# segasai/rvspecfit

Hardware: AMD Instinct MI355X
Metric: spectra/sec (CCF+chi2 grid) DESI 3-arm (higher is better)
Workload: dtype f64

## Files before the change

rvspecfit_amd/csrc/ccf_fft.hip:

```cpp
#include "common.h"

#define XC_NT 512
#define XC_NTW(n2) ((n2) >> 3)

__device__ __forceinline__ double2 cmul(double2 a, double2 b) {
  return make_double2(a.x * b.x - a.y * b.y, a.x * b.y + a.y * b.x);
}
__device__ __forceinline__ double2 cadd(double2 a, double2 b) {
  return make_double2(a.x + b.x, a.y + b.y);
}
__device__ __forceinline__ double2 csub(double2 a, double2 b) {
  return make_double2(a.x - b.x, a.y - b.y);
}
template <int SIGN>
__device__ __forceinline__ double2 cmuli(double2 a) {
  return (SIGN > 0) ? make_double2(-a.y, a.x) : make_double2(a.y, -a.x);
}

__host__ __device__ inline int xc_plan(int log2n, int *rad) {
  int n = 0, l = log2n;
  while (l >= 3) {
    rad[n++] = 8;
    l -= 3;
  }
// ... 44 lines not shown
  a[4] = csub(e0, o0);
  a[1] = cadd(e1, w1o);
  a[5] = csub(e1, w1o);
  a[2] = cadd(e2, w2o);
  a[6] = csub(e2, w2o);
  a[3] = cadd(e3, w3o);
  a[7] = csub(e3, w3o);
}

template <int SIGN>
__device__ __forceinline__ double2 twid(const double2 *__restrict__ tw, int e,
                                        int nfft) {
  const int half = nfft >> 1;
  double2 w = (e < half) ? tw[e] : tw[e - half];
  if (e >= half) {
    w.x = -w.x;
    w.y = -w.y;
  }
  if (SIGN < 0) w.y = -w.y;
  return w;
}

#ifdef RVS_XC_TIMING
__device__ unsigned long long xc_dbg[16];
#define XC_T(i)                                        \
  do {                                                 \
    __syncthreads();                                   \
    if (threadIdx.x == 0) {                            \
      const unsigned long long t_ = wall_clock64();    \
      atomicAdd(&xc_dbg[i], t_ - t_prev);              \
      t_prev = t_;                                     \
    }                                                  \
  } while (0)
extern "C" int rvs_dbg_read_xc(unsigned long long *out) {
  return hipMemcpyFromSymbol(out, HIP_SYMBOL(xc_dbg), sizeof(xc_dbg)) ==
                 hipSuccess
             ? 0
             : -1;
}
#else
#define XC_T(i)
#endif

template <int NT>
__device__ __forceinline__ void xc_fill_twiddles(double2 *a, int n2,
                                                 const double2 *__restrict__ tw) {
  const int ntw = XC_NTW(n2);
  if ((ntw & 63) == 0) {
    const int lane = threadIdx.x & 63;
    for (int i0 = (threadIdx.x >> 6) * 64; i0 < ntw; i0 += NT) {
      __builtin_amdgcn_global_load_lds(
          (const __attribute__((address_space(1))) void *)(tw + 2 * (i0 + lane)),
          (__attribute__((address_space(3))) void *)(a + n2 + i0), 16, 0, 0);
    }
    return;
  }
  for (int i = threadIdx.x; i < ntw; i += NT) a[n2 + i] = tw[2 * i];
}

struct XcMasks {
  unsigned g, b0, b7;
};
template <int NT>
__device__ __forceinline__ XcMasks xc_load_masks(const uint8_t *__restrict__ prune,
                                                 int n2) {
  XcMasks m = {0u, 0u, 0u};
  if (prune && (n2 >> 3) <= NT) {
    const int t = threadIdx.x, B = t >> 3;
    if (t < (n2 >> 3)) m.g = prune[(n2 >> 6) + t];
    if (B < (n2 >> 6)) {
      m.b0 = prune[(n2 >> 6) + 8 * B];
      m.b7 = prune[(n2 >> 6) + 8 * B + 7];
    }
  }
// ... 128 lines not shown
          const double2 w2 = cmul(w1, w1), w3 = cmul(w2, w1);
          v1 = cmul(v1, w1);
          v2 = cmul(v2, w2);
          v3 = cmul(v3, w3);
        }
        a[base] = v0;
        a[base + Mp] = v1;
        a[base + 2 * Mp] = v2;
        a[base + 3 * Mp] = v3;
      } else {
        const double2 v0 = a[base], v1 = a[base + Mp];
        double2 d = csub(v0, v1);
        if (Mp > 1) d = cmul(d, twid<SIGN>(tw, r << tws, nfft));
        a[base] = cadd(v0, v1);
        a[base + Mp] = d;
      }
    }
    lgM = lgMp;
  }
  __syncthreads();
}

__device__ __forceinline__ int fft_pos(int f, int log2n) {
  int pos = 0, lgm = log2n;
  while (lgm > 0) {
    const int lgr = lgm >= 3 ? 3 : lgm;
    lgm -= lgr;
    pos += (f & ((1 << lgr) - 1)) << lgm;
    f >>= lgr;
  }
  return pos;
}

__global__ void __launch_bounds__(XC_NT)
    ccf_rfft_kernel(const double *__restrict__ proc_spec,
                    const double *__restrict__ proc_ivar, int nfft, int log2n,
                    const double2 *__restrict__ tw, double2 *__restrict__ work) {
  extern __shared__ double2 fa[];
  const int b = blockIdx.x, which = blockIdx.y, tid = threadIdx.x;
  const int n2 = nfft >> 1;
  const double *ps = proc_spec + (int64_t)b * nfft;
  const double *pi = proc_ivar + (int64_t)b * nfft;
  xc_fill_twiddles<XC_NT>(fa, n2, tw);
  for (int n = tid; n < n2; n += XC_NT) {
    double x0, x1;
    if (which == 0) {
      x0 = ps[2 * n] * pi[2 * n];
      x1 = ps[2 * n + 1] * pi[2 * n + 1];
    } else {
      x0 = pi[2 * n];
      x1 = pi[2 * n + 1];
    }
    fa[n] = make_double2(x0, x1);
  }
  fft_lds<-1, XC_NT>(fa, log2n, tw);
  double2 *out = work + ((int64_t)b * 2 + which) * (n2 + 1);
  for (int k = tid; k <= n2; k += XC_NT) {
    double2 X;
    if (k == 0 || k == n2) {
      const double2 z0 = fa[0];
      X = make_double2(k == 0 ? z0.x + z0.y : z0.x - z0.y, 0.0);
    } else {
      const double2 zk = fa[fft_pos(k, log2n)];
      const double2 zm = fa[fft_pos(n2 - k, log2n)];
      const double2 e = make_double2(zk.x + zm.x, zk.y - zm.y);
      const double2 d = make_double2(zk.x - zm.x, zk.y + zm.y);
      const double2 q = cmul(twid<-1>(tw, k, nfft), d);
      X = make_double2(0.5 * (e.x + q.y), 0.5 * (e.y - q.x));
    }
    out[k] = make_double2(X.x, -X.y);
  }
}

#define XB_NT 512

__device__ __forceinline__ bool xc_job(unsigned bid, int T, int B, int G, int &b,
                                       int &t) {
  const int xcd = bid & 7;
  const int slot = bid >> 3;
  const int tt = slot % G;
  const int q = slot / G;
  b = q % B;
  const int g = q / B;
  t = xcd + 8 * (g * G + tt);
  return t < T;
}
__host__ inline int64_t xc_nblocks(int T, int B, int G) {
  const int ntx = (T + 7) >> 3;
  const int ngrp = (ntx + G - 1) / G;
  return 8ll * ngrp * G * B;
}
__host__ inline int xc_group(int T, int nfft) {
  const int64_t per_t = 2ll * ((nfft >> 1) + 1) * 16;
  if (per_t * T <= (16ll << 20)) return 0;
#ifndef XC_GROUP_BYTES
#define XC_GROUP_BYTES (2ll << 20)
#endif
  int G = (int)(XC_GROUP_BYTES / per_t);
  const int ntx = (T + 7) >> 3;
  if (G < 1) G = 1;
  if (G > ntx) G = ntx;
// ... 169 lines not shown
#define XW_NT 1024
#define XW_HALF 512

template <int SIGN, int LOG2N>
__device__ __forceinline__ void xw_pass(double2 *a, const double2 *T1, int p, int t,
                                        const double2 *Tc = nullptr) {
  const int lgM = LOG2N - 3 * p, lgMp = lgM - 3, Mp = 1 << lgMp;
  const int tws = LOG2N + 1 - lgM;
  const int blk = t >> lgMp, r = t & (Mp - 1);
  const int base = (blk << lgM) + r;
  double2 v[8];
#pragma unroll
  for (int j = 0; j < 8; j++) v[j] = a[base + Mp * j];
  dft8<SIGN>(v);
  if (Mp > 1) {
    double2 w1 = Tc ? Tc[r] : T1[r << (tws - 1)];
    if (SIGN < 0) w1.y = -w1.y;
    v[1] = cmul(v[1], w1);
    const double2 w2 = cmul(w1, w1);
    v[2] = cmul(v[2], w2);
    double2 wc = cmul(w2, w1);
    v[3] = cmul(v[3], wc);
    const double2 w4 = cmul(w2, w2);
    v[4] = cmul(v[4], w4);
    v[7] = cmul(v[7], cmul(w4, wc));
    wc = cmul(w4, w1);
    v[5] = cmul(v[5], wc);
    v[6] = cmul(v[6], cmul(w4, w2));
  }
#pragma unroll
  for (int q = 0; q < 8; q++) a[base + Mp * q] = v[q];
}

template <int LOG2N, bool RATIO>
__global__ void __launch_bounds__(XW_NT)
    ccf_xcorr_ws_kernel(const double2 *__restrict__ work,
                        const double2 *__restrict__ tfft,
                        const double2 *__restrict__ tfft2, int T,
                        const double2 *__restrict__ tw,
                        const int32_t *__restrict__ lag_pos,
                        const double *__restrict__ lag_vel, int nlag,
                        const int32_t *__restrict__ ilo,
                        const double *__restrict__ vgrid, int nvel, double beta,
                        const uint8_t *__restrict__ prune,
                        double *__restrict__ chisq) {
  extern __shared__ double2 fa[];
  constexpr int log2n = LOG2N, n2 = 1 << LOG2N, nfft = 2 * n2, npair = n2 / 2;
  constexpr int NPP = npair / XW_HALF;
  constexpr bool P12 = (LOG2N == 12);
  static_assert(LOG2N == 12 || LOG2N == 11, "plans 8,8,8,8 and 8,8,8,4 only");
  auto img = [&](int i) -> double2 * { return fa + (i & 1) * n2; };
  const double2 *T1 = fa + 2 * n2;
  double *c0 = reinterpret_cast<double *>(fa + 2 * n2 + XC_NTW(n2));
  double2 *T1c = fa + 2 * n2 + XC_NTW(n2) + ((nlag + 1) >> 1);
  double *cA = reinterpret_cast<double *>(T1c + 73);
  const int TI = RATIO ? 2 * T : T;
  const int b = blockIdx.x, tid = threadIdx.x;
  const bool producer = tid >= XW_HALF;
  const int pt = tid & (XW_HALF - 1);
  const double inv_n = 1.0 / nfft;
  if (P12 && tid < 72)
    T1c[tid] = tid < 64 ? tw[2 * (tid << 3)] : tw[2 * ((tid - 64) << (log2n - 6))];
  xc_fill_twiddles<XW_NT>(fa + n2, n2, tw);
  XcMasks pmask = {0u, 0u, 0u};
  bool bad = !P12;
  if (P12 && !producer) {
    pmask = xc_load_masks<XW_HALF>(prune, n2);
    const int pos8 = pt & 7;
    const unsigned m = pmask.g;
    bad = m != 0 && !((pos8 == 0 && m == 0x01u) || (pos8 == 7 && m == 0x80u));
  }
  const bool fold = !__syncthreads_or(bad);
  const double2 *Sc = work + ((int64_t)b * 2) * (n2 + 1);
  const double2 *Vc = Sc + (n2 + 1);
  typedef int v4i_t __attribute__((ext_vector_type(4)));
  auto ld = [](const __amdgpu_buffer_rsrc_t &r, int off) {
    const v4i_t v = __builtin_amdgcn_raw_buffer_load_b128(r, off, 0, 0);
    return make_double2(__hiloint2double(v.y, v.x), __hiloint2double(v.w, v.z));
  };
  const int nbytes = (n2 + 1) * 16;
  if (producer) {
    double2 Sk[NPP], Vk[NPP], Sm[NPP], Vm[NPP];
#pragma unroll
    for (int u = 0; u < NPP; u++) {
      const int k = 1 + pt + u * XW_HALF, m = n2 - k;
      Sk[u] = Sc[k], Vk[u] = Vc[k], Sm[u] = Sc[m], Vm[u] = Vc[m];
    }
    const __amdgpu_buffer_rsrc_t rT = __builtin_amdgcn_make_buffer_rsrc(
        (void *)tw, 0, (npair + 1) * 16, 0x00020000);
    double2 op[2][5];
    auto issue = [&](int t, int u, double2 *o) {
      const int tt = RATIO ? (t >> 1) : t;
      const __amdgpu_buffer_rsrc_t rF = __builtin_amdgcn_make_buffer_rsrc(
          (void *)(((RATIO && (t & 1)) ? tfft2 : tfft) + (int64_t)tt * (n2 + 1)), 0,
          nbytes, 0x00020000);
      const __amdgpu_buffer_rsrc_t rF2 = __builtin_amdgcn_make_buffer_rsrc(
          (void *)(tfft2 + (int64_t)tt * (n2 + 1)), 0, nbytes, 0x00020000);
      int ptv = pt;
      asm volatile("" : "+v"(ptv));
      const int k = 1 + ptv + u * XW_HALF;
      const int ok = k * 16, om = (n2 - k) * 16;
      if (RATIO) {
        o[0] = ld(rF, ok);
        o[2] = ld(rF, om);
      } else {
        o[0] = ld(rF, ok), o[1] = ld(rF2, ok);
        o[2] = ld(rF, om), o[3] = ld(rF2, om);
      }
      o[4] = ld(rT, ok);
    };
    double2 dc[4];
    auto form = [&](double2 *dst, int u, const double2 *o, int tcur) {
      int ptv = pt;
      asm volatile("" : "+v"(ptv));
      const int k = 1 + ptv + u * XW_HALF, m = n2 - k;
      double2 Xk, Xm;
      if (RATIO) {
        const bool second = (tcur & 1) != 0;
        Xk = cmul(o[0], second ? Vk[u] : Sk[u]);
        Xm = cmul(o[2], second ? Vm[u] : Sm[u]);
      } else {
        const double2 p1 = cmul(o[0], Sk[u]), p2 = cmul(o[1], Vk[u]);
        Xk = make_double2(p2.x - 2 * p1.x, p2.y - 2 * p1.y);
        const double2 q1 = cmul(o[2], Sm[u]), q2 = cmul(o[3], Vm[u]);
        Xm = make_double2(q2.x - 2 * q1.x, q2.y - 2 * q1.y);
      }
      const double2 e = make_double2(Xk.x + Xm.x, Xk.y - Xm.y);
      const double2 d = make_double2(Xk.x - Xm.x, Xk.y + Xm.y);
      const double2 q = cmul(o[4], d);
      dst[k] = make_double2(e.x - q.y, e.y + q.x);
      if (m != k) dst[m] = make_double2(e.x + q.y, -e.y + q.x);
      if (u == NPP - 1 && ptv == 0) {
        double xk, xm;
        if (RATIO) {
          const bool second = (tcur & 1) != 0;
          xk = cmul(second ? dc[1] : dc[0], second ? Vc[0] : Sc[0]).x;
          xm = cmul(second ? dc[3] : dc[2], second ? Vc[n2] : Sc[n2]).x;
        } else {
          const double2 a1 = cmul(dc[0], Sc[0]), a2 = cmul(dc[1], Vc[0]);
          const double2 b1 = cmul(dc[2], Sc[n2]), b2 = cmul(dc[3], Vc[n2]);
          xk = a2.x - 2 * a1.x, xm = b2.x - 2 * b1.x;
        }
        dst[0] = make_double2(xk + xm, xk - xm);
      }
    };
    const int nbar = (P12 && fold) ? 4 : 5;
    issue(0, 0, op[0]);
    if (NPP == 2) issue(0, 1, op[1]);
    for (int it = -1; it < TI; it++) {
      const int tn = it + 1;
      if (tn < TI) {
        double2 *dst = img(tn);
        {
          const int tt = RATIO ? (tn >> 1) : tn;
          const double2 *Fp = tfft + (int64_t)tt * (n2 + 1);
          const double2 *F2p = tfft2 + (int64_t)tt * (n2 + 1);
          dc[0] = Fp[0], dc[1] = F2p[0], dc[2] = Fp[n2], dc[3] = F2p[n2];
        }
        if (NPP == 2) {
#pragma unroll
          for (int u = 0; u < 2; u++) {
            form(dst, u, op[u], tn);
            if (tn + 1 < TI) issue(tn + 1, u, op[u]);
            __syncthreads();
          }
        } else {
#pragma unroll
          for (int u = 0; u < NPP; u++) {
            if (u + 1 < NPP)
              issue(tn, u + 1, op[(u + 1) & 1]);
            else if (tn + 1 < TI)
              issue(tn + 1, 0, op[(u + 1) & 1]);
            form(dst, u, op[u & 1], tn);
            __syncthreads();
          }
        }
        for (int q = NPP; q < nbar; q++) __syncthreads();
      } else {
        for (int q = 0; q < nbar; q++) __syncthreads();
      }
    }
    return;
  }
  const int tvx = min(pt, nvel - 1);
  const int pre_pos = lag_pos[min(pt, nlag - 1)];
  const int pre_lo = ilo[tvx];
  const double pre_xg = vgrid[tvx];
  const double pre_x0 = lag_vel[pre_lo], pre_x1 = lag_vel[pre_lo + 1];
  for (int it = -1; it < TI; it++) {
    if (it < 0) {
      const int nbar = (P12 && fold) ? 4 : 5;
      for (int q = 0; q < nbar; q++) __syncthreads();
      continue;
    }
    double2 *a = img(it);
    double *out = chisq + ((int64_t)b * T + (RATIO ? (it >> 1) : it)) * nvel;
    double pre_old = 0;
    if (beta != 0.0) pre_old = out[tvx];
    if (pt < (n2 >> 3)) xw_pass<1, LOG2N>(a, T1, 0, pt);
    __syncthreads();
    if (pt < (n2 >> 3)) xw_pass<1, LOG2N>(a, T1, 1, pt, P12 ? T1c : nullptr);
    __syncthreads();
    if (!P12) {
      if (pt < (n2 >> 3)) xw_pass<1, LOG2N>(a, T1, 2, pt);
      __syncthreads();
      {
        const int base = pt << 2;
        double2 v0 = a[base], v1 = a[base + 1], v2 = a[base + 2], v3 = a[base + 3];
        dft4<1>(v0, v1, v2, v3);
        a[base] = v0, a[base + 1] = v1, a[base + 2] = v2, a[base + 3] = v3;
      }
      __syncthreads();
    } else if (fold) {
      const int s = pt & 7;
      const int B = pt >> 3;
      const unsigned m0 = pmask.b0 & 1u, m63 = pmask.b7 >> 7;
      if (m0 | m63) {
        double2 v[8];
#pragma unroll
        for (int j = 0; j < 8; j++) v[j] = a[B * 64 + s + 8 * j];
        dft8<1>(v);
        double2 w = T1c[64 + s];
        w.y = -w.y;
        double2 x63 = cmul(v[7], w), x0 = v[0];
        auto sum8 = [](double x) {
          x += dpp_get<0xb1, 0xf, 0xf>(x);
          x += dpp_get<0x4e, 0xf, 0xf>(x);
          x += dpp_get<0x141, 0xf, 0xf>(x);
          return x;
        };
        if (m0) {
          x0.x = sum8(x0.x);
          x0.y = sum8(x0.y);
          if (s == 0) a[B * 64] = x0;
        }
        if (m63) {
          x63.x = sum8(x63.x);
          x63.y = sum8(x63.y);
          if (s == 0) a[B * 64 + 63] = x63;
        }
      }
      __syncthreads();
    } else {
      {
        const int blk = pt >> 3, r = pt & 7, base = (blk << 6) + r;
        const unsigned mask = prune[blk];
        if (mask != 0) {
          double2 v[8];
#pragma unroll
          for (int j = 0; j < 8; j++) v[j] = a[base + 8 * j];
          dft8<1>(v);
          double2 wp[8];
          wp[0] = make_double2(1.0, 0.0);
          wp[1] = T1[r << (log2n + 1 - 6 - 1)];
          wp[2] = cmul(wp[1], wp[1]);
          wp[3] = cmul(wp[2], wp[1]);
          wp[4] = cmul(wp[2], wp[2]);
          wp[7] = cmul(wp[4], wp[3]);
          wp[5] = cmul(wp[4], wp[1]);
          wp[6] = cmul(wp[4], wp[2]);
#pragma unroll
          for (int q = 0; q < 8; q++)
            if (mask & (1u << q))
              a[base + 8 * q] = (q == 0) ? v[0] : cmul(v[q], wp[q]);
        }
      }
      __syncthreads();
      {
        const unsigned mask = pmask.g;
        if (mask != 0) {
          const int base = pt << 3;
          double2 v[8];
#pragma unroll
          for (int j = 0; j < 8; j++) v[j] = a[base + j];
          dft8<1>(v);
#pragma unroll
          for (int q = 0; q < 8; q++)
            if (mask & (1u << q)) a[base + q] = v[q];
        }
      }
      __syncthreads();
    }
    if (RATIO) {
      if (pt < nlag) {
        const double c = reinterpret_cast<const double *>(a)[pre_pos] * inv_n;
        if (it & 1)
          c0[pt] = -cA[pt] * cA[pt] / c;
        else
          cA[pt] = c;
      }
    } else if (pt < nlag) {
      c0[pt] = reinterpret_cast<const double *>(a)[pre_pos] * inv_n;
    }
    __syncthreads();
    if ((!RATIO || (it & 1)) && pt < nvel) {
      const double sl = (c0[pre_lo + 1] - c0[pre_lo]) / (pre_x1 - pre_x0);
      const double val = sl * (pre_xg - pre_x0) + c0[pre_lo];
      out[pt] = (beta != 0.0) ? beta * pre_old + val : val;
    }
  }
}

__global__ void __launch_bounds__(XW_NT)
    ccf_xcorr_ws2_kernel(const double2 *__restrict__ work,
                         const double2 *__restrict__ tfft,
                         const double2 *__restrict__ tfft2, int T,
                         const double2 *__restrict__ tw,
                         const int32_t *__restrict__ lag_pos,
                         const double *__restrict__ lag_vel, int nlag,
                         const int32_t *__restrict__ ilo,
                         const double *__restrict__ vgrid, int nvel, double beta,
                         double *__restrict__ chisq) {
  extern __shared__ double2 fa[];
  constexpr int LOG2N = 11, n2 = 1 << LOG2N, nfft = 2 * n2, npair = n2 / 2;
  constexpr int NBAR = 5;
  auto img = [&](int i, int j) -> double2 * { return fa + (((i & 1) << 1) + j) * n2; };
  const double2 *T1 = fa + 4 * n2;
  double *c0 = reinterpret_cast<double *>(fa + 4 * n2 + XC_NTW(n2));
  const int b = blockIdx.x, tid = threadIdx.x;
  const bool producer = tid >= XW_HALF;
  const int pt = tid & (XW_HALF - 1);
  const double inv_n = 1.0 / nfft;
  xc_fill_twiddles<XW_NT>(fa + 3 * n2, n2, tw);
  const double2 *Sc = work + ((int64_t)b * 2) * (n2 + 1);
  const double2 *Vc = Sc + (n2 + 1);
  typedef int v4i_t __attribute__((ext_vector_type(4)));
  auto ld = [](const __amdgpu_buffer_rsrc_t &r, int off) {
    const v4i_t v = __builtin_amdgcn_raw_buffer_load_b128(r, off, 0, 0);
    return make_double2(__hiloint2double(v.y, v.x), __hiloint2double(v.w, v.z));
  };
  const int nbytes = (n2 + 1) * 16;
  const int NIT = (T + 1) >> 1;
  __syncthreads();
  if (producer) {
    double2 Sk[2], Vk[2], Sm[2], Vm[2];
#pragma unroll
    for (int u = 0; u < 2; u++) {
      const int k = 1 + pt + u * XW_HALF, m = n2 - k;
      Sk[u] = Sc[k], Vk[u] = Vc[k], Sm[u] = Sc[m], Vm[u] = Vc[m];
    }
    const __amdgpu_buffer_rsrc_t rT = __builtin_amdgcn_make_buffer_rsrc(
        (void *)tw, 0, (npair + 1) * 16, 0x00020000);
    double2 op[2][5];
    auto issue = [&](int t, int u, double2 *o) {
      const __amdgpu_buffer_rsrc_t rF = __builtin_amdgcn_make_buffer_rsrc(
          (void *)(tfft + (int64_t)t * (n2 + 1)), 0, nbytes, 0x00020000);
      const __amdgpu_buffer_rsrc_t rF2 = __builtin_amdgcn_make_buffer_rsrc(
          (void *)(tfft2 + (int64_t)t * (n2 + 1)), 0, nbytes, 0x00020000);
      const int k = 1 + pt + u * XW_HALF;
      const int ok = k * 16, om = (n2 - k) * 16;
      o[0] = ld(rF, ok), o[1] = ld(rF2, ok);
      o[2] = ld(rF, om), o[3] = ld(rF2, om);
      o[4] = ld(rT, ok);
    };
    auto form = [&](double2 *dst, int t, int u, const double2 *o) {
      const int k = 1 + pt + u * XW_HALF, m = n2 - k;
      const double2 p1 = cmul(o[0], Sk[u]), p2 = cmul(o[1], Vk[u]);
      const double2 Xk = make_double2(p2.x - 2 * p1.x, p2.y - 2 * p1.y);
      const double2 q1 = cmul(o[2], Sm[u]), q2 = cmul(o[3], Vm[u]);
      const double2 Xm = make_double2(q2.x - 2 * q1.x, q2.y - 2 * q1.y);
      const double2 e = make_double2(Xk.x + Xm.x, Xk.y - Xm.y);
      const double2 d = make_double2(Xk.x - Xm.x, Xk.y + Xm.y);
      const double2 q = cmul(o[4], d);
      dst[k] = make_double2(e.x - q.y, e.y + q.x);
      if (m != k) dst[m] = make_double2(e.x + q.y, -e.y + q.x);
      if (u == 1 && pt == 0) {
        const double2 *Fp = tfft + (int64_t)t * (n2 + 1);
        const double2 *F2p = tfft2 + (int64_t)t * (n2 + 1);
        const double2 a1 = cmul(Fp[0], Sc[0]), a2 = cmul(F2p[0], Vc[0]);
        const double2 b1 = cmul(Fp[n2], Sc[n2]), b2 = cmul(F2p[n2], Vc[n2]);
        const double xk = a2.x - 2 * a1.x, xm = b2.x - 2 * b1.x;
        dst[0] = make_double2(xk + xm, xk - xm);
      }
    };
    auto tq = [&](int i, int q) { return min(2 * i + (q >> 1), T - 1); };
    issue(tq(0, 0), 0, op[0]);
    for (int it = -1; it < NIT; it++) {
      const int in = it + 1;
      if (in < NIT) {
#pragma unroll
        for (int q = 0; q < 4; q++) {
          if (q + 1 < 4)
            issue(tq(in, q + 1), (q + 1) & 1, op[(q + 1) & 1]);
          else if (in + 1 < NIT)
            issue(tq(in + 1, 0), 0, op[(q + 1) & 1]);
          form(img(in, q >> 1), tq(in, q), q & 1, op[q & 1]);
          __syncthreads();
        }
        __syncthreads();
      } else {
        for (int q = 0; q < NBAR; q++) __syncthreads();
      }
    }
    return;
  }
  const int j = pt >> 8, bt = pt & 255;
  int pre_pos[1], dummy = 0;
  (void)dummy;
  pre_pos[0] = lag_pos[min(pt, nlag - 1)];
  const int tvx = min(pt, nvel - 1);
  const int pre_lo = ilo[tvx];
  const double pre_xg = vgrid[tvx];
  const double pre_x0 = lag_vel[pre_lo], pre_x1 = lag_vel[pre_lo + 1];
  for (int it = -1; it < NIT; it++) {
    if (it < 0) {
      for (int q = 0; q < NBAR; q++) __syncthreads();
      continue;
    }
    double2 *a = img(it, j);
    const int t0 = 2 * it, t1 = min(2 * it + 1, T - 1);
    const bool two = (2 * it + 1 < T);
    double *out0 = chisq + ((int64_t)b * T + t0) * nvel;
    double *out1 = chisq + ((int64_t)b * T + t1) * nvel;
    double old0 = 0, old1 = 0;
    if (beta != 0.0) {
      old0 = out0[tvx];
      old1 = out1[tvx];
    }
    xw_pass<1, LOG2N>(a, T1, 0, bt);
    __syncthreads();
    xw_pass<1, LOG2N>(a, T1, 1, bt);
    __syncthreads();
    xw_pass<1, LOG2N>(a, T1, 2, bt);
    __syncthreads();
#pragma unroll
    for (int h = 0; h < 2; h++) {
      const int base = (bt + 256 * h) << 2;
      double2 v0 = a[base], v1 = a[base + 1], v2 = a[base + 2], v3 = a[base + 3];
// ... 19 lines not shown
    }
  }
}

extern "C" int rvs_ccf_xcorr(const double *proc_spec, const double *proc_ivar,
                             int nfft, int B, const double *tfft,
                             const double *tfft2, int T, const double *twid_,
                             int continuum, const int32_t *lag_pos,
                             const double *lag_vel, int nlag, const int32_t *ilo,
                             const double *vgrid, int nvel, double beta,
                             const uint8_t *prune, double *chisq, double *work,
                             void *stream) {
  int log2n = 0;
  while ((2 << log2n) < nfft) log2n++;
  if ((2 << log2n) != nfft || nfft < 64 || nfft > 16384) return RVS_E_ARG;
  if (B < 1 || T < 1 || T > 65535 || nlag < 2 || nvel < 1) return RVS_E_ARG;
  const int n2 = nfft >> 1;
  const size_t shm1 = sizeof(double2) * (size_t)(n2 + XC_NTW(n2));
  const size_t shm2 = shm1 + sizeof(double) * 2 * (size_t)nlag;
  if (shm2 > 159 * 1024) return RVS_E_ARG;
  hipStream_t st = rvs_stream(stream);
  const double2 *tw = reinterpret_cast<const double2 *>(twid_);
  static bool attr_set = false;
  if (!attr_set) {
    (void)hipFuncSetAttribute((const void *)ccf_rfft_kernel,
                              hipFuncAttributeMaxDynamicSharedMemorySize,
                              159 * 1024);
    (void)hipFuncSetAttribute((const void *)ccf_xcorr_kernel,
                              hipFuncAttributeMaxDynamicSharedMemorySize,
                              159 * 1024);
    (void)hipGetLastError();
    attr_set = true;
  }
  hipLaunchKernelGGL(ccf_rfft_kernel, dim3(B, 2), dim3(XC_NT), shm1, st,
                     proc_spec, proc_ivar, nfft, log2n, tw,
                     reinterpret_cast<double2 *>(work));
  RVS_LAUNCH_CHECK();
  const int G = xc_group(T, nfft);
  {
    const bool ws_on = rvs_opt(RVS_OPT_XC_WS) != 0;
    const bool p12 = (nfft == 8192 && prune), p11 = (nfft == 4096);
    if (ws_on && (p12 || p11) && nlag <= XW_HALF && nvel <= XW_HALF && T >= 2) {
      static bool ws_attr = false;
      if (!ws_attr) {
        (void)hipFuncSetAttribute((const void *)ccf_xcorr_ws_kernel<12, false>,
                                  hipFuncAttributeMaxDynamicSharedMemorySize,
                                  159 * 1024);
        (void)hipFuncSetAttribute((const void *)ccf_xcorr_ws_kernel<12, true>,
                                  hipFuncAttributeMaxDynamicSharedMemorySize,
                                  159 * 1024);
        (void)hipFuncSetAttribute((const void *)ccf_xcorr_ws_kernel<11, true>,
                                  hipFuncAttributeMaxDynamicSharedMemorySize,
                                  159 * 1024);
        (void)hipFuncSetAttribute((const void *)ccf_xcorr_ws2_kernel,
                                  hipFuncAttributeMaxDynamicSharedMemorySize,
                                  159 * 1024);
        (void)hipGetLastError();
        ws_attr = true;
      }
      const size_t shmw = sizeof(double2) * (size_t)(2 * n2 + XC_NTW(n2)) +
                          sizeof(double) * (size_t)nlag +
                          sizeof(double2) * (72 + 1) +
                          (continuum ? 0 : sizeof(double) * (size_t)nlag);
#define RVS_XW_ARGS                                                                 \
  reinterpret_cast<const double2 *>(work), reinterpret_cast<const double2 *>(tfft),  \
      reinterpret_cast<const double2 *>(tfft2), T, tw, lag_pos, lag_vel, nlag, ilo,  \
      vgrid, nvel, beta, prune, chisq
      if (!continuum) {
        if (p12)
          hipLaunchKernelGGL((ccf_xcorr_ws_kernel<12, true>), dim3(B), dim3(XW_NT), shmw,
                             st, RVS_XW_ARGS);
        else
          hipLaunchKernelGGL((ccf_xcorr_ws_kernel<11, true>), dim3(B), dim3(XW_NT), shmw,
                             st, RVS_XW_ARGS);
        RVS_LAUNCH_CHECK();
        return 0;
      }
      if (p12)
        hipLaunchKernelGGL((ccf_xcorr_ws_kernel<12, false>), dim3(B), dim3(XW_NT), shmw, st,
                           reinterpret_cast<const double2 *>(work),
                           reinterpret_cast<const double2 *>(tfft),
                           reinterpret_cast<const double2 *>(tfft2), T, tw, lag_pos,
                           lag_vel, nlag, ilo, vgrid, nvel, beta, prune, chisq);
      else
        hipLaunchKernelGGL(ccf_xcorr_ws2_kernel, dim3(B), dim3(XW_NT),
                           sizeof(double2) * (size_t)(4 * n2 + XC_NTW(n2)) +
                               sizeof(double) * 2 * (size_t)nlag,
                           st, reinterpret_cast<const double2 *>(work),
                           reinterpret_cast<const double2 *>(tfft),
                           reinterpret_cast<const double2 *>(tfft2), T, tw, lag_pos,
                           lag_vel, nlag, ilo, vgrid, nvel, beta, chisq);
      RVS_LAUNCH_CHECK();
      return 0;
    }
  }
  const int bmax = G ? (int)(0x7fffffffll / xc_nblocks(T, 1, G)) : 65535;
  for (int b0 = 0; b0 < B; b0 += bmax) {
    const int nb = (B - b0 < bmax) ? (B - b0) : bmax;
    const dim3 grid = G ? dim3((unsigned)xc_nblocks(T, nb, G)) : dim3(T, nb);
    hipLaunchKernelGGL(
        ccf_xcorr_kernel, grid, dim3(XB_NT), shm2, st,
        reinterpret_cast<const double2 *>(work) + (int64_t)b0 * 2 * (n2 + 1),
        nfft, log2n, reinterpret_cast<const double2 *>(tfft),
        reinterpret_cast<const double2 *>(tfft2), T, tw, continuum, lag_pos,
        lag_vel, nlag, ilo, vgrid, nvel, beta, prune,
        chisq + (int64_t)b0 * T * nvel, nb, G);
    RVS_LAUNCH_CHECK();
  }
  return 0;
}
```

Measured before the change: 77560.

## Cut barriers in warp-specialized xcorr kernel for the folded FFT path

Restructures the producer/consumer pipeline of the warp-specialized cross-correlation kernel. The folded 4096-point path now writes the pruned lag outputs straight from the DPP reductions through a precomputed shared-memory lag map, which drops the later passes and reduces the barriers per template from four to two. Other changes: the producer keeps its post-processing twiddles in registers instead of reloading them, the DC/Nyquist term moves to a consumer thread, and the chi-square row store is deferred by one iteration to overlap it with the next FFT. Optional s_memtime instrumentation is added behind a compile flag. This adds complexity and depends on a delicate barrier-count match between producer and consumer.

New measurement: 78710, median of 6. 1.5% higher.

```diff
diff --git a/rvspecfit_amd/csrc/ccf_fft.hip b/rvspecfit_amd/csrc/ccf_fft.hip
--- a/rvspecfit_amd/csrc/ccf_fft.hip
+++ b/rvspecfit_amd/csrc/ccf_fft.hip
@@ -572,6 +572,40 @@
   for (int q = 0; q < 8; q++) a[base + Mp * q] = v[q];
 }
 
+__device__ __forceinline__ constexpr int xw_nbar(bool folded) { return folded ? 2 : 5; }
+#ifdef RVS_XC_TIMING
+__device__ unsigned long long xw_dbg[2][5][2];
+#define XW_SYNC(q)                                               \
+  do {                                                           \
+    const unsigned t0_ = (unsigned)__builtin_amdgcn_s_memtime(); \
+    __syncthreads();                                             \
+    const unsigned t1_ = (unsigned)__builtin_amdgcn_s_memtime(); \
+    if (pt == 0) {                                               \
+      xw_cnt[(producer * 5 + (q)) * 2] += t0_ - xw_t;            \
+      xw_cnt[(producer * 5 + (q)) * 2 + 1] += t1_ - t0_;         \
+    }                                                            \
+    xw_t = t1_;                                                  \
+  } while (0)
+#define XW_DUMP()                                                           \
+  do {                                                                      \
+    if (pt == 0)                                                            \
+      for (int i_ = 0; i_ < 10; i_++)                                       \
+        atomicAdd(&xw_dbg[producer][i_ >> 1][i_ & 1],                       \
+                  (unsigned long long)xw_cnt[producer * 10 + i_]);          \
+  } while (0)
+extern "C" int rvs_dbg_read_xw(unsigned long long *out) {
+  return hipMemcpyFromSymbol(out, HIP_SYMBOL(xw_dbg), sizeof(xw_dbg)) == hipSuccess ? 0
+                                                                                    : -1;
+}
+#else
+#define XW_SYNC(q) __syncthreads()
+#define XW_DUMP()
+#endif
+__host__ __device__ constexpr int xw_lagd2(int nlag) { return (nlag + 1) >> 1; }
+__host__ __device__ constexpr int xw_tail(int n2, int nlag) {
+  return 2 * xw_lagd2(nlag) + 72 + (((n2 >> 6) * 4 * 2 + 15) >> 4);
+}
+
 template <int LOG2N, bool RATIO>
 __global__ void __launch_bounds__(XW_NT)
     ccf_xcorr_ws_kernel(const double2 *__restrict__ work,
@@ -592,8 +626,9 @@
   auto img = [&](int i) -> double2 * { return fa + (i & 1) * n2; };
   const double2 *T1 = fa + 2 * n2;
   double *c0 = reinterpret_cast<double *>(fa + 2 * n2 + XC_NTW(n2));
-  double2 *T1c = fa + 2 * n2 + XC_NTW(n2) + ((nlag + 1) >> 1);
-  double *cA = reinterpret_cast<double *>(T1c + 73);
+  double2 *T1c = fa + 2 * n2 + XC_NTW(n2) + xw_lagd2(nlag);
+  double *cA = reinterpret_cast<double *>(T1c + 72);
+  int16_t *lmap = reinterpret_cast<int16_t *>(T1c + 72 + xw_lagd2(nlag));
   const int TI = RATIO ? 2 * T : T;
   const int b = blockIdx.x, tid = threadIdx.x;
   const bool producer = tid >= XW_HALF;
@@ -604,13 +639,22 @@
   xc_fill_twiddles<XW_NT>(fa + n2, n2, tw);
   XcMasks pmask = {0u, 0u, 0u};
   bool bad = !P12;
+  int pre_pos = 0;
+  if (!producer) pre_pos = lag_pos[min(pt, nlag - 1)];
   if (P12 && !producer) {
+    if (pt < 4 * (n2 >> 6)) lmap[pt] = -1;
     pmask = xc_load_masks<XW_HALF>(prune, n2);
     const int pos8 = pt & 7;
     const unsigned m = pmask.g;
     bad = m != 0 && !((pos8 == 0 && m == 0x01u) || (pos8 == 7 && m == 0x80u));
   }
+#ifdef RVS_XC_TIMING
+  __shared__ unsigned xw_cnt[20];
+  if (tid < 20) xw_cnt[tid] = 0;
+  unsigned xw_t = (unsigned)__builtin_amdgcn_s_memtime();
+#endif
   const bool fold = !__syncthreads_or(bad);
+  const int nbar = xw_nbar(P12 && fold);
   const double2 *Sc = work + ((int64_t)b * 2) * (n2 + 1);
   const double2 *Vc = Sc + (n2 + 1);
   typedef int v4i_t __attribute__((ext_vector_type(4)));
@@ -626,9 +670,13 @@
       const int k = 1 + pt + u * XW_HALF, m = n2 - k;
       Sk[u] = Sc[k], Vk[u] = Vc[k], Sm[u] = Sc[m], Vm[u] = Vc[m];
     }
-    const __amdgpu_buffer_rsrc_t rT = __builtin_amdgcn_make_buffer_rsrc(
-        (void *)tw, 0, (npair + 1) * 16, 0x00020000);
-    double2 op[2][5];
+    double2 op[2][4];
+    double2 twr[NPP];
+#pragma unroll
+    for (int u = 0; u < NPP; u++) {
+      twr[u] = tw[1 + pt + u * XW_HALF];
+      asm volatile("" : "+v"(twr[u].x), "+v"(twr[u].y));
+    }
     auto issue = [&](int t, int u, double2 *o) {
       const int tt = RATIO ? (t >> 1) : t;
       const __amdgpu_buffer_rsrc_t rF = __builtin_amdgcn_make_buffer_rsrc(
@@ -647,9 +695,7 @@
         o[0] = ld(rF, ok), o[1] = ld(rF2, ok);
         o[2] = ld(rF, om), o[3] = ld(rF2, om);
       }
-      o[4] = ld(rT, ok);
     };
-    double2 dc[4];
     auto form = [&](double2 *dst, int u, const double2 *o, int tcur) {
       int ptv = pt;
       asm volatile("" : "+v"(ptv));
@@ -667,91 +713,92 @@
       }
       const double2 e = make_double2(Xk.x + Xm.x, Xk.y - Xm.y);
       const double2 d = make_double2(Xk.x - Xm.x, Xk.y + Xm.y);
-      const double2 q = cmul(o[4], d);
+      const double2 q = cmul(twr[u], d);
       dst[k] = make_double2(e.x - q.y, e.y + q.x);
       if (m != k) dst[m] = make_double2(e.x + q.y, -e.y + q.x);
-      if (u == NPP - 1 && ptv == 0) {
-        double xk, xm;
-        if (RATIO) {
-          const bool second = (tcur & 1) != 0;
-          xk = cmul(second ? dc[1] : dc[0], second ? Vc[0] : Sc[0]).x;
-          xm = cmul(second ? dc[3] : dc[2], second ? Vc[n2] : Sc[n2]).x;
-        } else {
-          const double2 a1 = cmul(dc[0], Sc[0]), a2 = cmul(dc[1], Vc[0]);
-          const double2 b1 = cmul(dc[2], Sc[n2]), b2 = cmul(dc[3], Vc[n2]);
-          xk = a2.x - 2 * a1.x, xm = b2.x - 2 * b1.x;
-        }
-        dst[0] = make_double2(xk + xm, xk - xm);
-      }
     };
-    const int nbar = (P12 && fold) ? 4 : 5;
+    const bool pairs = nbar < NPP;
     issue(0, 0, op[0]);
-    if (NPP == 2) issue(0, 1, op[1]);
-    for (int it = -1; it < TI; it++) {
-      const int tn = it + 1;
-      if (tn < TI) {
-        double2 *dst = img(tn);
-        {
-          const int tt = RATIO ? (tn >> 1) : tn;
-          const double2 *Fp = tfft + (int64_t)tt * (n2 + 1);
-          const double2 *F2p = tfft2 + (int64_t)tt * (n2 + 1);
-          dc[0] = Fp[0], dc[1] = F2p[0], dc[2] = Fp[n2], dc[3] = F2p[n2];
-        }
-        if (NPP == 2) {
-#pragma unroll
-          for (int u = 0; u < 2; u++) {
-            form(dst, u, op[u], tn);
-            if (tn + 1 < TI) issue(tn + 1, u, op[u]);
-            __syncthreads();
-          }
-        } else {
-#pragma unroll
-          for (int u = 0; u < NPP; u++) {
-            if (u + 1 < NPP)
-              issue(tn, u + 1, op[(u + 1) & 1]);
-            else if (tn + 1 < TI)
-              issue(tn + 1, 0, op[(u + 1) & 1]);
-            form(dst, u, op[u & 1], tn);
-            __syncthreads();
-          }
-        }
-        for (int q = NPP; q < nbar; q++) __syncthreads();
-      } else {
-        for (int q = 0; q < nbar; q++) __syncthreads();
-      }
-    }
+    issue(0, 1, op[1]);
+    for (int tn = 0; tn < TI; tn++) {
+      double2 *dst = img(tn);
+#pragma unroll
+      for (int u = 0; u < NPP; u++) {
+        form(dst, u, op[u & 1], tn);
+        if (u + 2 < NPP)
+          issue(tn, u + 2, op[u & 1]);
+        else
+          issue(min(tn + 1, TI - 1), u + 2 - NPP, op[u & 1]);
+        if (!pairs || (u & 1)) XW_SYNC(pairs ? u >> 1 : u);
+      }
+      for (int q = pairs ? NPP / 2 : NPP; q < nbar; q++) XW_SYNC(q);
+    }
+    for (int q = 0; q < nbar; q++) XW_SYNC(q);
+    XW_DUMP();
     return;
   }
+  const bool folded = P12 && fold;
   const int tvx = min(pt, nvel - 1);
-  const int pre_pos = lag_pos[min(pt, nlag - 1)];
   const int pre_lo = ilo[tvx];
   const double pre_xg = vgrid[tvx];
   const double pre_x0 = lag_vel[pre_lo], pre_x1 = lag_vel[pre_lo + 1];
-  for (int it = -1; it < TI; it++) {
-    if (it < 0) {
-      const int nbar = (P12 && fold) ? 4 : 5;
-      for (int q = 0; q < nbar; q++) __syncthreads();
-      continue;
-    }
+  auto put_lag = [&](int l, double c, int it) {
+    if (!RATIO)
+      c0[l] = c;
+    else if (it & 1)
+      c0[l] = -cA[l] * cA[l] / c;
+    else
+      cA[l] = c;
+  };
+  auto store_row = [&](int t, double old) {
+    if (pt < nvel) {
+      const double sl = (c0[pre_lo + 1] - c0[pre_lo]) / (pre_x1 - pre_x0);
+      const double val = sl * (pre_xg - pre_x0) + c0[pre_lo];
+      chisq[((int64_t)b * T + t) * nvel + pt] = (beta != 0.0) ? beta * old + val : val;
+    }
+  };
+  auto form_dc = [&](int tcur) {
+    if (pt != XW_HALF - 1 || tcur >= TI) return;
+    const int tt = RATIO ? (tcur >> 1) : tcur;
+    const double2 *Fp = tfft + (int64_t)tt * (n2 + 1);
+    const double2 *F2p = tfft2 + (int64_t)tt * (n2 + 1);
+    const double2 dc[4] = {Fp[0], F2p[0], Fp[n2], F2p[n2]};
+    double xk, xm;
+    if (RATIO) {
+      const bool second = (tcur & 1) != 0;
+      xk = cmul(second ? dc[1] : dc[0], second ? Vc[0] : Sc[0]).x;
+      xm = cmul(second ? dc[3] : dc[2], second ? Vc[n2] : Sc[n2]).x;
+    } else {
+      const double2 a1 = cmul(dc[0], Sc[0]), a2 = cmul(dc[1], Vc[0]);
+      const double2 b1 = cmul(dc[2], Sc[n2]), b2 = cmul(dc[3], Vc[n2]);
+      xk = a2.x - 2 * a1.x, xm = b2.x - 2 * b1.x;
+    }
+    img(tcur)[0] = make_double2(xk + xm, xk - xm);
+  };
+  form_dc(0);
+  if (folded && pt < nlag) {
+    const unsigned e = (unsigned)pre_pos >> 1, r = e & 63u;
+    if (e < (unsigned)n2 && (r == 0u || r == 63u))
+      lmap[4 * (e >> 6) + (r ? 2 : 0) + (pre_pos & 1)] = (int16_t)pt;
+  }
+  for (int q = 0; q < nbar; q++) XW_SYNC(q);
+  uint2 slots = make_uint2(~0u, ~0u);
+  if (folded) slots = reinterpret_cast<const uint2 *>(lmap)[pt >> 3];
+  double pre_old = 0;
+  for (int it = 0; it < TI; it++) {
     double2 *a = img(it);
-    double *out = chisq + ((int64_t)b * T + (RATIO ? (it >> 1) : it)) * nvel;
-    double pre_old = 0;
-    if (beta != 0.0) pre_old = out[tvx];
+    const int tt = RATIO ? (it >> 1) : it;
+    const bool head = !RATIO || !(it & 1), tail = !RATIO || (it & 1);
+    form_dc(it + 1);
+    if (folded && head && it > 0) store_row(tt - 1, pre_old);
+    if (beta != 0.0 && (head || !folded)) pre_old = chisq[((int64_t)b * T + tt) * nvel + tvx];
     if (pt < (n2 >> 3)) xw_pass<1, LOG2N>(a, T1, 0, pt);
-    __syncthreads();
+    XW_SYNC(0);
     if (pt < (n2 >> 3)) xw_pass<1, LOG2N>(a, T1, 1, pt, P12 ? T1c : nullptr);
-    __syncthreads();
-    if (!P12) {
-      if (pt < (n2 >> 3)) xw_pass<1, LOG2N>(a, T1, 2, pt);
-      __syncthreads();
-      {
-        const int base = pt << 2;
-        double2 v0 = a[base], v1 = a[base + 1], v2 = a[base + 2], v3 = a[base + 3];
-        dft4<1>(v0, v1, v2, v3);
-        a[base] = v0, a[base + 1] = v1, a[base + 2] = v2, a[base + 3] = v3;
-      }
-      __syncthreads();
-    } else if (fold) {
+    if (folded) {
+      __builtin_amdgcn_fence(__ATOMIC_RELEASE, "wavefront");
+      __builtin_amdgcn_wave_barrier();
+      __builtin_amdgcn_fence(__ATOMIC_ACQUIRE, "wavefront");
       const int s = pt & 7;
       const int B = pt >> 3;
       const unsigned m0 = pmask.b0 & 1u, m63 = pmask.b7 >> 7;
@@ -769,16 +816,34 @@
           x += dpp_get<0x141, 0xf, 0xf>(x);
           return x;
         };
+        auto put = [&](unsigned slot, double x) {
+          if (s == 0 && slot != 0xffffu) put_lag((int)slot, x * inv_n, it);
+        };
         if (m0) {
           x0.x = sum8(x0.x);
           x0.y = sum8(x0.y);
-          if (s == 0) a[B * 64] = x0;
+          put(slots.x & 0xffffu, x0.x);
+          put(slots.x >> 16, x0.y);
         }
         if (m63) {
           x63.x = sum8(x63.x);
           x63.y = sum8(x63.y);
-          if (s == 0) a[B * 64 + 63] = x63;
+          put(slots.y & 0xffffu, x63.x);
+          put(slots.y >> 16, x63.y);
         }
+      }
+      XW_SYNC(1);
+      continue;
+    }
+    XW_SYNC(1);
+    if (!P12) {
+      if (pt < (n2 >> 3)) xw_pass<1, LOG2N>(a, T1, 2, pt);
+      XW_SYNC(2);
+      {
+        const int base = pt << 2;
+        double2 v0 = a[base], v1 = a[base + 1], v2 = a[base + 2], v3 = a[base + 3];
+        dft4<1>(v0, v1, v2, v3);
+        a[base] = v0, a[base + 1] = v1, a[base + 2] = v2, a[base + 3] = v3;
       }
       __syncthreads();
     } else {
@@ -821,24 +886,12 @@
       }
       __syncthreads();
     }
-    if (RATIO) {
-      if (pt < nlag) {
-        const double c = reinterpret_cast<const double *>(a)[pre_pos] * inv_n;
-        if (it & 1)
-          c0[pt] = -cA[pt] * cA[pt] / c;
-        else
-          cA[pt] = c;
-      }
-    } else if (pt < nlag) {
-      c0[pt] = reinterpret_cast<const double *>(a)[pre_pos] * inv_n;
-    }
+    if (pt < nlag) put_lag(pt, reinterpret_cast<const double *>(a)[pre_pos] * inv_n, it);
     __syncthreads();
-    if ((!RATIO || (it & 1)) && pt < nvel) {
-      const double sl = (c0[pre_lo + 1] - c0[pre_lo]) / (pre_x1 - pre_x0);
-      const double val = sl * (pre_xg - pre_x0) + c0[pre_lo];
-      out[pt] = (beta != 0.0) ? beta * pre_old + val : val;
-    }
-  }
+    if (tail) store_row(tt, pre_old);
+  }
+  if (folded) store_row(T - 1, pre_old);
+  XW_DUMP();
 }
 
 __global__ void __launch_bounds__(XW_NT)
@@ -1045,10 +1098,8 @@
         (void)hipGetLastError();
         ws_attr = true;
       }
-      const size_t shmw = sizeof(double2) * (size_t)(2 * n2 + XC_NTW(n2)) +
-                          sizeof(double) * (size_t)nlag +
-                          sizeof(double2) * (72 + 1) +
-                          (continuum ? 0 : sizeof(double) * (size_t)nlag);
+      const size_t shmw =
+          sizeof(double2) * (size_t)(2 * n2 + XC_NTW(n2) + xw_tail(n2, nlag));
 #define RVS_XW_ARGS                                                                 \
   reinterpret_cast<const double2 *>(work), reinterpret_cast<const double2 *>(tfft),  \
       reinterpret_cast<const double2 *>(tfft2), T, tw, lag_pos, lag_vel, nlag, ilo,  \
```

## Fuse forward real FFT into warp-specialized xcorr kernel, dropping separate rfft launch

Applied to the files above, without the earlier changes.

The forward real FFTs of spec*ivar and ivar now run inside the warp-specialized cross-correlation kernels. Each half of the block transforms one image in LDS, and the producer unfolds the half-spectra directly from a swizzled LDS layout. This removes a separate kernel launch and the global round trip through the work buffer. In exchange, the FFT now sits on the critical path of each xcorr block, which adds LDS traffic and register pressure. Timing probe macros are also added.

Measured after the change: 77240 before, 78250 after (median of 6 runs). 1.3% higher.

```diff
diff --git a/rvspecfit_amd/csrc/ccf_fft.hip b/rvspecfit_amd/csrc/ccf_fft.hip
--- a/rvspecfit_amd/csrc/ccf_fft.hip
+++ b/rvspecfit_amd/csrc/ccf_fft.hip
@@ -100,6 +100,11 @@
       t_prev = t_;                                     \
     }                                                  \
   } while (0)
+#define XC_T0() unsigned long long t_prev = wall_clock64()
+#define XC_TEND(i)                                                       \
+  do {                                                                   \
+    if (threadIdx.x == 0) atomicAdd(&xc_dbg[i], wall_clock64() - t_prev); \
+  } while (0)
 extern "C" int rvs_dbg_read_xc(unsigned long long *out) {
   return hipMemcpyFromSymbol(out, HIP_SYMBOL(xc_dbg), sizeof(xc_dbg)) ==
                  hipSuccess
@@ -108,6 +113,8 @@
 }
 #else
 #define XC_T(i)
+#define XC_T0()
+#define XC_TEND(i)
 #endif
 
 template <int NT>
@@ -302,6 +309,13 @@
   return pos;
 }
 
+__device__ __forceinline__ double2 rfft_unfold(double2 zk, double2 zm, double2 w) {
+  const double2 e = make_double2(zk.x + zm.x, zk.y - zm.y);
+  const double2 d = make_double2(zk.x - zm.x, zk.y + zm.y);
+  const double2 q = cmul(w, d);
+  return make_double2(0.5 * (e.x + q.y), 0.5 * (e.y - q.x));
+}
+
 __global__ void __launch_bounds__(XC_NT)
     ccf_rfft_kernel(const double *__restrict__ proc_spec,
                     const double *__restrict__ proc_ivar, int nfft, int log2n,
@@ -333,10 +347,7 @@
     } else {
       const double2 zk = fa[fft_pos(k, log2n)];
       const double2 zm = fa[fft_pos(n2 - k, log2n)];
-      const double2 e = make_double2(zk.x + zm.x, zk.y - zm.y);
-      const double2 d = make_double2(zk.x - zm.x, zk.y + zm.y);
-      const double2 q = cmul(twid<-1>(tw, k, nfft), d);
-      X = make_double2(0.5 * (e.x + q.y), 0.5 * (e.y - q.x));
+      X = rfft_unfold(zk, zm, twid<-1>(tw, k, nfft));
     }
     out[k] = make_double2(X.x, -X.y);
   }
@@ -572,9 +583,102 @@
   for (int q = 0; q < 8; q++) a[base + Mp * q] = v[q];
 }
 
+template <int LOG2N>
+__device__ __forceinline__ int xw_swz(int p) {
+  constexpr int sh = (LOG2N == 12) ? 6 : 5;
+  return p ^ ((p >> sh) & 15);
+}
+
+template <int LOG2N>
+__device__ __forceinline__ void xw_pack(double2 *fa, const double *__restrict__ ps,
+                                        const double *__restrict__ pi) {
+  constexpr int n2 = 1 << LOG2N, NPT = n2 / XW_NT;
+  double2 s[NPT], v[NPT];
+#pragma unroll
+  for (int j = 0; j < NPT; j++) {
+    const int n = threadIdx.x + j * XW_NT;
+    s[j] = make_double2(ps[2 * n], ps[2 * n + 1]);
+    v[j] = make_double2(pi[2 * n], pi[2 * n + 1]);
+  }
+#pragma unroll
+  for (int j = 0; j < NPT; j++) {
+    const int n = threadIdx.x + j * XW_NT;
+    fa[n] = make_double2(s[j].x * v[j].x, s[j].y * v[j].y);
+    fa[n2 + n] = v[j];
+  }
+}
+
+template <int LOG2N>
+__device__ __forceinline__ void xw_forward(double2 *fa, const double2 *T1,
+                                           const double2 *Tc) {
+  constexpr int n2 = 1 << LOG2N;
+  const int pt = threadIdx.x & (XW_HALF - 1);
+  double2 *a = fa + (threadIdx.x / XW_HALF) * n2;
+#pragma unroll
+  for (int p = 0; p < 3; p++) {
+    if (pt < (n2 >> 3)) xw_pass<-1, LOG2N>(a, T1, p, pt, p == 1 ? Tc : nullptr);
+    __syncthreads();
+  }
+  if (LOG2N == 12) {
+    const int base = pt << 3;
+    double2 v[8];
+#pragma unroll
+    for (int j = 0; j < 8; j++) v[j] = a[base + j];
+    dft8<-1>(v);
+#pragma unroll
+    for (int q = 0; q < 8; q++) a[xw_swz<LOG2N>(base + q)] = v[q];
+  } else {
+    const int base = pt << 2;
+    double2 v0 = a[base], v1 = a[base + 1], v2 = a[base + 2], v3 = a[base + 3];
+    dft4<-1>(v0, v1, v2, v3);
+    a[xw_swz<LOG2N>(base)] = v0, a[xw_swz<LOG2N>(base + 1)] = v1;
+    a[xw_swz<LOG2N>(base + 2)] = v2, a[xw_swz<LOG2N>(base + 3)] = v3;
+  }
+  __syncthreads();
+}
+
+__device__ __forceinline__ double xw_uniform(double x) {
+  return __hiloint2double(__builtin_amdgcn_readfirstlane(__double2hiint(x)),
+                          __builtin_amdgcn_readfirstlane(__double2loint(x)));
+}
+
+template <int LOG2N, int NPP>
+__device__ __forceinline__ void xw_unfold(const double2 *fa,
+                                          const double2 *__restrict__ tw, int pt,
+                                          double2 (&Sk)[NPP], double2 (&Vk)[NPP],
+                                          double2 (&Sm)[NPP], double2 (&Vm)[NPP],
+                                          double (&dcn)[4]) {
+  constexpr int n2 = 1 << LOG2N, nfft = 2 * n2;
+  double2 wk[NPP], wm[NPP];
+#pragma unroll
+  for (int u = 0; u < NPP; u++) {
+    const int k = 1 + pt + u * XW_HALF;
+    wk[u] = twid<-1>(tw, k, nfft), wm[u] = twid<-1>(tw, n2 - k, nfft);
+  }
+#pragma unroll
+  for (int u = 0; u < NPP; u++) {
+    const int k = 1 + pt + u * XW_HALF;
+    const int pk = xw_swz<LOG2N>(fft_pos(k, LOG2N));
+    const int pm = xw_swz<LOG2N>(fft_pos(n2 - k, LOG2N));
+    const double2 sk = fa[pk], sm = fa[pm], vk = fa[n2 + pk], vm = fa[n2 + pm];
+    double2 X = rfft_unfold(sk, sm, wk[u]);
+    Sk[u] = make_double2(X.x, -X.y);
+    X = rfft_unfold(sm, sk, wm[u]);
+    Sm[u] = make_double2(X.x, -X.y);
+    X = rfft_unfold(vk, vm, wk[u]);
+    Vk[u] = make_double2(X.x, -X.y);
+    X = rfft_unfold(vm, vk, wm[u]);
+    Vm[u] = make_double2(X.x, -X.y);
+  }
+  const double2 s0 = fa[0], v0 = fa[n2];
+  dcn[0] = xw_uniform(s0.x + s0.y), dcn[1] = xw_uniform(s0.x - s0.y);
+  dcn[2] = xw_uniform(v0.x + v0.y), dcn[3] = xw_uniform(v0.x - v0.y);
+}
+
 template <int LOG2N, bool RATIO>
 __global__ void __launch_bounds__(XW_NT)
-    ccf_xcorr_ws_kernel(const double2 *__restrict__ work,
+    ccf_xcorr_ws_kernel(const double *__restrict__ proc_spec,
+                        const double *__restrict__ proc_ivar,
                         const double2 *__restrict__ tfft,
                         const double2 *__restrict__ tfft2, int T,
                         const double2 *__restrict__ tw,
@@ -599,20 +703,26 @@
   const bool producer = tid >= XW_HALF;
   const int pt = tid & (XW_HALF - 1);
   const double inv_n = 1.0 / nfft;
-  if (P12 && tid < 72)
-    T1c[tid] = tid < 64 ? tw[2 * (tid << 3)] : tw[2 * ((tid - 64) << (log2n - 6))];
+  XC_T0();
+  const int tc = min(tid, 71);
+  const double2 t1c =
+      tw[P12 ? 2 * (tc < 64 ? tc << 3 : (tc - 64) << (log2n - 6)) : 0];
   xc_fill_twiddles<XW_NT>(fa + n2, n2, tw);
   XcMasks pmask = {0u, 0u, 0u};
+  if (P12 && !producer) pmask = xc_load_masks<XW_HALF>(prune, n2);
+  xw_pack<LOG2N>(fa, proc_spec + (int64_t)b * nfft, proc_ivar + (int64_t)b * nfft);
+  if (P12 && tid < 72) T1c[tid] = t1c;
+  asm volatile("" : "+v"(pmask.g), "+v"(pmask.b0), "+v"(pmask.b7));
   bool bad = !P12;
   if (P12 && !producer) {
-    pmask = xc_load_masks<XW_HALF>(prune, n2);
     const int pos8 = pt & 7;
     const unsigned m = pmask.g;
     bad = m != 0 && !((pos8 == 0 && m == 0x01u) || (pos8 == 7 && m == 0x80u));
   }
   const bool fold = !__syncthreads_or(bad);
-  const double2 *Sc = work + ((int64_t)b * 2) * (n2 + 1);
-  const double2 *Vc = Sc + (n2 + 1);
+  XC_T(3);
+  xw_forward<LOG2N>(fa, T1, P12 ? T1c : nullptr);
+  XC_T(4);
   typedef int v4i_t __attribute__((ext_vector_type(4)));
   auto ld = [](const __amdgpu_buffer_rsrc_t &r, int off) {
     const v4i_t v = __builtin_amdgcn_raw_buffer_load_b128(r, off, 0, 0);
@@ -621,11 +731,12 @@
   const int nbytes = (n2 + 1) * 16;
   if (producer) {
     double2 Sk[NPP], Vk[NPP], Sm[NPP], Vm[NPP];
-#pragma unroll
-    for (int u = 0; u < NPP; u++) {
-      const int k = 1 + pt + u * XW_HALF, m = n2 - k;
-      Sk[u] = Sc[k], Vk[u] = Vc[k], Sm[u] = Sc[m], Vm[u] = Vc[m];
-    }
+    double dcn[4];
+    xw_unfold<LOG2N, NPP>(fa, tw, pt, Sk, Vk, Sm, Vm, dcn);
+    const double2 Sc0 = make_double2(dcn[0], -0.0), Scn = make_double2(dcn[1], -0.0);
+    const double2 Vc0 = make_double2(dcn[2], -0.0), Vcn = make_double2(dcn[3], -0.0);
+    __syncthreads();
+    XC_T(5);
     const __amdgpu_buffer_rsrc_t rT = __builtin_amdgcn_make_buffer_rsrc(
         (void *)tw, 0, (npair + 1) * 16, 0x00020000);
     double2 op[2][5];
@@ -674,11 +785,11 @@
         double xk, xm;
         if (RATIO) {
           const bool second = (tcur & 1) != 0;
-          xk = cmul(second ? dc[1] : dc[0], second ? Vc[0] : Sc[0]).x;
-          xm = cmul(second ? dc[3] : dc[2], second ? Vc[n2] : Sc[n2]).x;
+          xk = cmul(second ? dc[1] : dc[0], second ? Vc0 : Sc0).x;
+          xm = cmul(second ? dc[3] : dc[2], second ? Vcn : Scn).x;
         } else {
-          const double2 a1 = cmul(dc[0], Sc[0]), a2 = cmul(dc[1], Vc[0]);
-          const double2 b1 = cmul(dc[2], Sc[n2]), b2 = cmul(dc[3], Vc[n2]);
+          const double2 a1 = cmul(dc[0], Sc0), a2 = cmul(dc[1], Vc0);
+          const double2 b1 = cmul(dc[2], Scn), b2 = cmul(dc[3], Vcn);
           xk = a2.x - 2 * a1.x, xm = b2.x - 2 * b1.x;
         }
         dst[0] = make_double2(xk + xm, xk - xm);
@@ -722,6 +833,8 @@
     }
     return;
   }
+  __syncthreads();
+  XC_T(5);
   const int tvx = min(pt, nvel - 1);
   const int pre_pos = lag_pos[min(pt, nlag - 1)];
   const int pre_lo = ilo[tvx];
@@ -839,10 +952,12 @@
       out[pt] = (beta != 0.0) ? beta * pre_old + val : val;
     }
   }
+  XC_TEND(6);
 }
 
 __global__ void __launch_bounds__(XW_NT)
-    ccf_xcorr_ws2_kernel(const double2 *__restrict__ work,
+    ccf_xcorr_ws2_kernel(const double *__restrict__ proc_spec,
+                         const double *__restrict__ proc_ivar,
                          const double2 *__restrict__ tfft,
                          const double2 *__restrict__ tfft2, int T,
                          const double2 *__restrict__ tw,
@@ -862,8 +977,7 @@
   const int pt = tid & (XW_HALF - 1);
   const double inv_n = 1.0 / nfft;
   xc_fill_twiddles<XW_NT>(fa + 3 * n2, n2, tw);
-  const double2 *Sc = work + ((int64_t)b * 2) * (n2 + 1);
-  const double2 *Vc = Sc + (n2 + 1);
+  xw_pack<LOG2N>(fa, proc_spec + (int64_t)b * nfft, proc_ivar + (int64_t)b * nfft);
   typedef int v4i_t __attribute__((ext_vector_type(4)));
   auto ld = [](const __amdgpu_buffer_rsrc_t &r, int off) {
     const v4i_t v = __builtin_amdgcn_raw_buffer_load_b128(r, off, 0, 0);
@@ -872,13 +986,14 @@
   const int nbytes = (n2 + 1) * 16;
   const int NIT = (T + 1) >> 1;
   __syncthreads();
+  xw_forward<LOG2N>(fa, T1, nullptr);
   if (producer) {
     double2 Sk[2], Vk[2], Sm[2], Vm[2];
-#pragma unroll
-    for (int u = 0; u < 2; u++) {
-      const int k = 1 + pt + u * XW_HALF, m = n2 - k;
-      Sk[u] = Sc[k], Vk[u] = Vc[k], Sm[u] = Sc[m], Vm[u] = Vc[m];
-    }
+    double dcn[4];
+    xw_unfold<LOG2N, 2>(fa, tw, pt, Sk, Vk, Sm, Vm, dcn);
+    const double2 Sc0 = make_double2(dcn[0], -0.0), Scn = make_double2(dcn[1], -0.0);
+    const double2 Vc0 = make_double2(dcn[2], -0.0), Vcn = make_double2(dcn[3], -0.0);
+    __syncthreads();
     const __amdgpu_buffer_rsrc_t rT = __builtin_amdgcn_make_buffer_rsrc(
         (void *)tw, 0, (npair + 1) * 16, 0x00020000);
     double2 op[2][5];
@@ -907,8 +1022,8 @@
       if (u == 1 && pt == 0) {
         const double2 *Fp = tfft + (int64_t)t * (n2 + 1);
         const double2 *F2p = tfft2 + (int64_t)t * (n2 + 1);
-        const double2 a1 = cmul(Fp[0], Sc[0]), a2 = cmul(F2p[0], Vc[0]);
-        const double2 b1 = cmul(Fp[n2], Sc[n2]), b2 = cmul(F2p[n2], Vc[n2]);
+        const double2 a1 = cmul(Fp[0], Sc0), a2 = cmul(F2p[0], Vc0);
+        const double2 b1 = cmul(Fp[n2], Scn), b2 = cmul(F2p[n2], Vcn);
         const double xk = a2.x - 2 * a1.x, xm = b2.x - 2 * b1.x;
         dst[0] = make_double2(xk + xm, xk - xm);
       }
@@ -934,6 +1049,7 @@
     }
     return;
   }
+  __syncthreads();
   const int j = pt >> 8, bt = pt & 255;
   int pre_pos[1], dummy = 0;
   (void)dummy;
@@ -1019,10 +1135,6 @@
     (void)hipGetLastError();
     attr_set = true;
   }
-  hipLaunchKernelGGL(ccf_rfft_kernel, dim3(B, 2), dim3(XC_NT), shm1, st,
-                     proc_spec, proc_ivar, nfft, log2n, tw,
-                     reinterpret_cast<double2 *>(work));
-  RVS_LAUNCH_CHECK();
   const int G = xc_group(T, nfft);
   {
     const bool ws_on = rvs_opt(RVS_OPT_XC_WS) != 0;
@@ -1046,11 +1158,11 @@
         ws_attr = true;
       }
       const size_t shmw = sizeof(double2) * (size_t)(2 * n2 + XC_NTW(n2)) +
-                          sizeof(double) * (size_t)nlag +
+                          sizeof(double2) * (size_t)((nlag + 1) >> 1) +
                           sizeof(double2) * (72 + 1) +
                           (continuum ? 0 : sizeof(double) * (size_t)nlag);
-#define RVS_XW_ARGS                                                                 \
-  reinterpret_cast<const double2 *>(work), reinterpret_cast<const double2 *>(tfft),  \
+#define RVS_XW_ARGS                                                                  \
+  proc_spec, proc_ivar, reinterpret_cast<const double2 *>(tfft),                     \
       reinterpret_cast<const double2 *>(tfft2), T, tw, lag_pos, lag_vel, nlag, ilo,  \
       vgrid, nvel, beta, prune, chisq
       if (!continuum) {
@@ -1065,15 +1177,12 @@
       }
       if (p12)
         hipLaunchKernelGGL((ccf_xcorr_ws_kernel<12, false>), dim3(B), dim3(XW_NT), shmw, st,
-                           reinterpret_cast<const double2 *>(work),
-                           reinterpret_cast<const double2 *>(tfft),
-                           reinterpret_cast<const double2 *>(tfft2), T, tw, lag_pos,
-                           lag_vel, nlag, ilo, vgrid, nvel, beta, prune, chisq);
+                           RVS_XW_ARGS);
       else
         hipLaunchKernelGGL(ccf_xcorr_ws2_kernel, dim3(B), dim3(XW_NT),
                            sizeof(double2) * (size_t)(4 * n2 + XC_NTW(n2)) +
                                sizeof(double) * 2 * (size_t)nlag,
-                           st, reinterpret_cast<const double2 *>(work),
+                           st, proc_spec, proc_ivar,
                            reinterpret_cast<const double2 *>(tfft),
                            reinterpret_cast<const double2 *>(tfft2), T, tw, lag_pos,
                            lag_vel, nlag, ilo, vgrid, nvel, beta, chisq);
@@ -1081,6 +1190,10 @@
       return 0;
     }
   }
+  hipLaunchKernelGGL(ccf_rfft_kernel, dim3(B, 2), dim3(XC_NT), shm1, st,
+                     proc_spec, proc_ivar, nfft, log2n, tw,
+                     reinterpret_cast<double2 *>(work));
+  RVS_LAUNCH_CHECK();
   const int bmax = G ? (int)(0x7fffffffll / xc_nblocks(T, 1, G)) : 65535;
   for (int b0 = 0; b0 < B; b0 += bmax) {
     const int nb = (B - b0 < bmax) ? (B - b0) : bmax;
```
